# yemam3/SAC-RCBF

Hardware: AMD Instinct MI355X
Metric: safe env steps/sec (dynamics+CBF-QP) at batch 65536, 1/2/4/8 MI355X (higher is better)
Workload: dtype f32 rows / f64 QP / f64 env

## Files before the change

### __graft_entry__.py

```python
import os
import subprocess
import sys

ROOT = os.path.dirname(os.path.abspath(__file__))
PKG = os.path.join(ROOT, "sac-rcbf_amd")
CSRC = os.path.join(PKG, "csrc")
LIB = os.path.join(PKG, "rcbf_amd", "librcbf_hip.so")
HIPCC = os.environ.get("HIPCC", "/opt/rocm/bin/hipcc")
HIP_FLAGS = ["--offload-arch=gfx950", "-O3", "-fPIC", "-std=c++17",
             "-fhip-fp32-correctly-rounded-divide-sqrt", "-Wno-unused-result",
             "-mllvm", "-amdgpu-kernarg-preload-count=16"]

for p in (ROOT, PKG):
    if p not in sys.path:
        sys.path.insert(0, p)


def _newer(target, sources):
    if not os.path.exists(target):
        return False
    t = os.path.getmtime(target)
    return all(os.path.getmtime(s) <= t for s in sources)


KERNEL_TUS = ["rcbf_qp.hip", "rcbf_qp_f64.hip", "rcbf_qp_bwd.hip", "rcbf_layer.hip", "rcbf_env.hip", "rcbf_cascade.hip",
              "rcbf_gp.hip", "rcbf_model.hip", "rcbf_aql.hip", "rcbf_steps_traj.hip", "rcbf_steps_term.hip", "rcbf_policy.hip"]
TU_FLAGS = {"rcbf_steps_term.hip": ["-mllvm", "-disable-machine-licm"]}
LLVM_BIN = "/opt/rocm/lib/llvm/bin"
STEPS_CO = os.path.join(PKG, "rcbf_amd", "librcbf_steps.co")
STEPS_TRAJ_CO = os.path.join(PKG, "rcbf_amd", "librcbf_steps_traj.co")
STEPS_TERM_CO = os.path.join(PKG, "rcbf_amd", "librcbf_steps_term.co")
POLICY_CO = os.path.join(PKG, "rcbf_amd", "librcbf_policy.co")


def _deps(path, seen=None):
    import re
    seen = set() if seen is None else seen
    if path in seen or not os.path.exists(path):
        return seen
    seen.add(path)
    for name in re.findall(r'^\s*#\s*include\s+"([^"]+)"', open(path).read(), re.M):
        for d in (os.path.dirname(path), CSRC, os.path.join(ROOT, "include")):
            cand = os.path.normpath(os.path.join(d, name))
            if os.path.exists(cand):
                _deps(cand, seen)
                break
    return seen
# ... 14 lines not shown
        obj = os.path.join(objdir, tu.replace(".hip", ".o"))
        objs.append(obj)
        if not force and _newer(obj, sorted(_deps(src))):
            continue
        cmd = [HIPCC, *HIP_FLAGS, *TU_FLAGS.get(tu, []), *defines, *inc, "-c", "-o", obj, src]
        print("[build]", " ".join(cmd), flush=True)
        procs.append(subprocess.Popen(cmd))
    if any(p.wait() != 0 for p in procs):
        raise RuntimeError("hipcc failed")
    open(flags_file, "w").write(flags)
    if out == LIB:
        extract_steps_co(os.path.join(objdir, "rcbf_env.o"), STEPS_CO)
        extract_steps_co(os.path.join(objdir, "rcbf_steps_traj.o"), STEPS_TRAJ_CO)
        extract_steps_co(os.path.join(objdir, "rcbf_steps_term.o"), STEPS_TERM_CO)
        extract_steps_co(os.path.join(objdir, "rcbf_policy.o"), POLICY_CO)
    if not procs and _newer(out, objs):
        return out
    cmd = [HIPCC, "--offload-arch=gfx950", "-shared", "-fPIC", "-o", out, *objs, "-L/opt/rocm/lib", "-lhsa-runtime64"]
    print("[build]", " ".join(cmd), flush=True)
    subprocess.run(cmd, check=True)
    return out


def extract_steps_co(obj, out):
    if _newer(out, [obj]):
        return out
    import tempfile
    with tempfile.TemporaryDirectory() as td:
        fat = os.path.join(td, "fatbin.bin")
        subprocess.run([os.path.join(LLVM_BIN, "llvm-objcopy"), "--dump-section=.hip_fatbin=" + fat, obj,
# ... 158 lines not shown
    print("[smoke] ok", flush=True)


if __name__ == "__main__":
    what = sys.argv[1] if len(sys.argv) > 1 else "build"
    if what == "variant":
        name, defs = sys.argv[2], sys.argv[3:]
        os.makedirs(os.path.join(ROOT, "build", "variants"), exist_ok=True)
        vdir = os.path.join(ROOT, "build", "variants")
        build_lib(force=True, out=os.path.join(vdir, f"librcbf_{name}.so"), defines=defs)
        objdir = os.path.join(ROOT, "build", "obj_" + "_".join(d.strip("-D").replace("=", "") for d in defs))
        extract_steps_co(os.path.join(objdir, "rcbf_env.o"), os.path.join(vdir, f"librcbf_{name}.co"))
        extract_steps_co(os.path.join(objdir, "rcbf_steps_traj.o"), os.path.join(vdir, f"librcbf_{name}_traj.co"))
        extract_steps_co(os.path.join(objdir, "rcbf_steps_term.o"), os.path.join(vdir, f"librcbf_{name}_term.co"))
        extract_steps_co(os.path.join(objdir, "rcbf_policy.o"), os.path.join(vdir, f"librcbf_{name}_policy.co"))
    else:
        {"build": build, "smoke": smoke, "build_oracle": lambda: build_oracle(force=True)}[what]()
```

### include/rcbf_hip.h

```cpp
#ifndef RCBF_HIP_H
#define RCBF_HIP_H

#include <stdint.h>
#include <hip/hip_runtime_api.h>

#ifdef __cplusplus
extern "C" {
#endif

#define RCBF_ABI_VERSION 13

#define RCBF_MODE_SIMULATED_CARS 0
#define RCBF_MODE_UNICYCLE 1

#define RCBF_FORM_DIFF 0
#define RCBF_FORM_CASCADE 1

#define RCBF_SOLVER_ACTIVE_SET 0
#define RCBF_SOLVER_PDIPM 1
#define RCBF_SOLVER_GI 2

#define RCBF_QP_OK 0
#define RCBF_QP_MAX_ITER 1
#define RCBF_QP_INFEASIBLE 2
// ... 228 lines not shown
#define RCBF_TRAJ_U 2
#define RCBF_TRAJ_REWARD 4
#define RCBF_TRAJ_COST 8
#define RCBF_TRAJ_DONE 16
#define RCBF_TRAJ_GOAL_MET 32
#define RCBF_TRAJ_STATUS 64
#define RCBF_TRAJ_TERM_OBS 128
#define RCBF_AQL_PROFILE 1
#define RCBF_AQL_FIRST_ACQUIRE_SYSTEM 2
#define RCBF_AQL_LAST_RELEASE_AGENT 4
#define RCBF_AQL_STUDY_MID_NOFENCE 8
#define RCBF_AQL_STUDY_MID_NOACQ 16
#define RCBF_AQL_STUDY_MID_NOREL 32
#define RCBF_AQL_PROFILE_ENDS 64
#define RCBF_AQL_PER_STEP 128
#define RCBF_AQL_SAFE_STEP_KERNARG_BYTES 408
#define RCBF_AQL_SAFE_STEPS_KERNARG_BYTES 408
#define RCBF_AQL_SAFE_STEPS_TRAJ_KERNARG_BYTES 424
#define RCBF_AQL_SAFE_STEPS_TERM_KERNARG_BYTES 432
#define RCBF_AQL_POLICY_STEP_KERNARG_BYTES 80
typedef struct rcbf_aql rcbf_aql;
typedef struct rcbf_aql_plan rcbf_aql_plan;
int rcbf_aql_open(int32_t device, const char* code_object, int32_t flags, rcbf_aql** out);
int rcbf_aql_close(rcbf_aql* q);
int rcbf_aql_kernel_count(const rcbf_aql* q);
int rcbf_aql_safe_step_plan(rcbf_aql* q, const rcbf_params* prm, int64_t B, int32_t K, double* x, double* aux,
                            int32_t* step, uint32_t* episode, const float* const* u_rl_seq, int32_t n_u_rl,
                            const float* mu, const float* sigma, int32_t prior_cols, float* obs_out, float* u_out,
                            float* reward, float* cost, uint8_t* done, uint8_t* goal_met, int32_t* status_out,
                            int32_t* fail_flag, int32_t auto_reset, uint64_t seed, int64_t env_offset,
// ... 12 lines not shown
                                 int32_t* status_out, int32_t* fail_flag, int32_t auto_reset, uint64_t seed,
                                 int64_t env_offset, uint64_t* span_out, int32_t flags, int32_t traj_mask,
                                 int64_t traj_pitch, float* term_obs, rcbf_aql_plan** out);
int rcbf_aql_closed_loop_plan(rcbf_aql* q, const rcbf_params* prm, int64_t B, int32_t K, double* x, double* aux,
                              int32_t* step, uint32_t* episode, float* u_rl_buf, const float* mu, const float* sigma,
                              int32_t prior_cols, float* obs_out, float* u_out, float* reward, float* cost,
                              uint8_t* done, uint8_t* goal_met, int32_t* status_out, int32_t* fail_flag,
                              int32_t auto_reset, uint64_t seed, int64_t env_offset, uint64_t* span_out,
                              int32_t flags, int32_t traj_mask, int64_t traj_pitch, float* term_obs,
                              const float* obs_in, const float* packed, int32_t n_o, int32_t n_u, int32_t hidden,
                              int32_t mode, uint64_t policy_seed, const uint64_t* counter_word,
                              int64_t policy_env_offset, rcbf_aql_plan** out);
int rcbf_aql_run(rcbf_aql_plan* plan, uint64_t timeout_us);
int rcbf_aql_plan_times(const rcbf_aql_plan* plan, uint64_t* start_end_ns);
int rcbf_aql_plan_dispatches(const rcbf_aql_plan* plan);
int rcbf_aql_plan_free(rcbf_aql_plan* plan);

#define RCBF_POLICY_MEAN 0
#define RCBF_POLICY_SAMPLE 1
int64_t rcbf_policy_packed_floats(int32_t n_o, int32_t n_u, int32_t hidden);
int rcbf_policy_act(const float* packed, int32_t n_o, int32_t n_u, int32_t hidden, int64_t B,
                    const float* obs, float* u_rl, int32_t mode, const float* z,
                    uint64_t seed, uint64_t counter, int64_t env_offset, hipStream_t stream);

const char* rcbf_version(void);
int32_t rcbf_abi_version(void);
int32_t rcbf_params_size(void);

#ifdef __cplusplus
}
// ... 3 lines not shown
```

### sac-rcbf_amd/csrc/rcbf_aql.hip

```cpp
#include <hip/hip_runtime.h>
#include <hsa/hsa.h>
#include <hsa/hsa_ext_amd.h>

#include <dlfcn.h>
#include <immintrin.h>
#include <time.h>

#include <atomic>
#include <cstddef>
#include <cstdio>
#include <cstring>
#include <string>
#include <vector>

#include "rcbf_hip.h"
#include "rcbf_policy_step.hpp"
#include "rcbf_safe_step.hpp"

namespace {

using namespace rcbf;

struct SafeStepArgs {
    int64_t B;
// ... 53 lines not shown
struct rcbf_aql {
    int device = -1;
    hsa_agent_t agent{};
    hsa_queue_t* queue = nullptr;
    hsa_code_object_reader_t reader{};
    hsa_code_object_reader_t reader_traj{};
    hsa_executable_t exe{};
    hsa_executable_t exe_traj{};
    hsa_code_object_reader_t reader_term{};
    hsa_executable_t exe_term{};
    bool have_reader = false, have_reader_traj = false, have_exe = false, have_exe_traj = false, hsa_up = false;
    bool have_reader_term = false, have_exe_term = false;
    hsa_code_object_reader_t reader_policy{};
    hsa_executable_t exe_policy{};
    bool have_reader_policy = false, have_exe_policy = false;
    std::vector<char> code, code_traj, code_term, code_policy;
    std::vector<KernelInfo> kernels;
    std::atomic<int> queue_error{0};
    int profiling = 0;
    bool fused = false;
    bool traj = false;
    bool term = false;
    bool policy = false;
};

struct rcbf_aql_plan {
    rcbf_aql* q = nullptr;
    int device = -1;
    int32_t K = 0;
    void* kernargs = nullptr;
    std::vector<hsa_kernel_dispatch_packet_t> pkt;
    std::vector<hsa_signal_t> sig;
    int profiled = 0;
};

namespace {

void queue_error_cb(hsa_status_t status, hsa_queue_t*, void* data) {
    auto* q = static_cast<rcbf_aql*>(data);
    q->queue_error.store((int)status);
}

struct AgentSearch {
    uint32_t bdf;
    uint32_t domain;
    hsa_agent_t found{};
    bool ok = false;
};
// ... 46 lines not shown
std::string safe_steps_prefix(int mode, int k, int bs) {
    char buf[128];
    snprintf(buf, sizeof buf, "_ZN4rcbf12k_safe_stepsILi%dELi%dELi%dEEEv", mode, k, bs);
    return buf;
}

std::string safe_steps_traj_prefix(int mode, int k, int bs) {
    char buf[128];
    snprintf(buf, sizeof buf, "_ZN4rcbf17k_safe_steps_trajILi%dELi%dELi%dEEEv", mode, k, bs);
    return buf;
}

std::string safe_steps_term_prefix(int mode, int k, int bs) {
    char buf[128];
    snprintf(buf, sizeof buf, "_ZN4rcbf17k_safe_steps_termILi%dELi%dELi%dEEEv", mode, k, bs);
    return buf;
}

std::string policy_step_prefix(bool sample, int nrb) {
    char buf[128];
    snprintf(buf, sizeof buf, "_ZN4rcbf13k_policy_stepILb%dELi%dEEEv", sample ? 1 : 0, nrb);
    return buf;
}

bool read_optional_code_object(const std::string& tpath, std::vector<char>& code);

bool read_side_code_object(const std::string& path, const char* suffix, std::vector<char>& code) {
    if (path.size() <= 3 || path.compare(path.size() - 3, 3, ".co") != 0) return true;
    return read_optional_code_object(path.substr(0, path.size() - 3) + suffix + ".co", code);
}
// ... 98 lines not shown
        if (hipGetDevice(&prev) != hipSuccess) prev = -1;
        if (prev != dev) (void)hipSetDevice(dev);
    }
    ~DeviceGuard() {
        if (prev >= 0) (void)hipSetDevice(prev);
    }
};

void destroy(rcbf_aql* q) {
    if (!q) return;
    if (q->queue) hsa_queue_destroy(q->queue);
    if (q->have_exe) hsa_executable_destroy(q->exe);
    if (q->have_exe_traj) hsa_executable_destroy(q->exe_traj);
    if (q->have_exe_term) hsa_executable_destroy(q->exe_term);
    if (q->have_exe_policy) hsa_executable_destroy(q->exe_policy);
    if (q->have_reader_policy) hsa_code_object_reader_destroy(q->reader_policy);
    if (q->have_reader) hsa_code_object_reader_destroy(q->reader);
    if (q->have_reader_traj) hsa_code_object_reader_destroy(q->reader_traj);
    if (q->have_reader_term) hsa_code_object_reader_destroy(q->reader_term);
    if (q->hsa_up) hsa_shut_down();
    delete q;
}

}

extern "C" {

int rcbf_aql_open(int32_t device, const char* code_object_path, int32_t flags, rcbf_aql** out) {
    if (!out) return RCBF_E_NULL;
    *out = nullptr;
// ... 21 lines not shown
    const bool read_ok = n > 0 && fread(q->code.data(), 1, (size_t)n, f) == (size_t)n;
    fclose(f);
    if (!read_ok) {
        delete q;
        return RCBF_E_BAD_SHAPE;
    }
    if (!read_side_code_object(path, "_traj", q->code_traj)) {
        delete q;
        return RCBF_E_BAD_SHAPE;
    }
    if (!read_side_code_object(path, "_term", q->code_term)) {
        delete q;
        return RCBF_E_BAD_SHAPE;
    }
    if (!read_optional_code_object(policy_code_object_path(path), q->code_policy)) {
        delete q;
        return RCBF_E_BAD_SHAPE;
    }
    int rc = hsa_rc(hsa_init());
    if (rc) {
        delete q;
        return rc;
    }
    q->hsa_up = true;
    hipDeviceProp_t prop;
    if (hipGetDeviceProperties(&prop, device) != hipSuccess) {
        destroy(q);
        return RCBF_E_HSA;
    }
    AgentSearch s{(uint32_t)((prop.pciBusID << 8) | (prop.pciDeviceID << 3)), (uint32_t)prop.pciDomainID};
// ... 42 lines not shown
    }
    if (!rc && !q->code_policy.empty()) {
        rc = hsa_rc(hsa_code_object_reader_create_from_memory(q->code_policy.data(), q->code_policy.size(),
                                                              &q->reader_policy));
        if (!rc) q->have_reader_policy = true;
        if (!rc)
            rc = hsa_rc(hsa_executable_create_alt(HSA_PROFILE_FULL, HSA_DEFAULT_FLOAT_ROUNDING_MODE_DEFAULT, nullptr,
                                                  &q->exe_policy));
        if (!rc) q->have_exe_policy = true;
        if (!rc)
            rc = hsa_rc(
                hsa_executable_load_agent_code_object(q->exe_policy, q->agent, q->reader_policy, nullptr, nullptr));
        if (!rc) rc = hsa_rc(hsa_executable_freeze(q->exe_policy, nullptr));
        if (!rc) rc = hsa_rc(hsa_executable_iterate_agent_symbols(q->exe_policy, q->agent, collect_kernel, q));
    }
    int n_steps = 0, n_fused = 0, n_traj = 0, n_term = 0;
    for (const auto& k : q->kernels) {
        if (k.name.compare(0, 21, "_ZN4rcbf11k_safe_step") == 0) {
            ++n_steps;
            if (k.kernarg_bytes != sizeof(SafeStepArgs) || k.private_bytes != 0) rc = RCBF_E_BAD_SHAPE;
        } else if (k.name.compare(0, 22, "_ZN4rcbf12k_safe_steps") == 0) {
            ++n_fused;
            if (k.kernarg_bytes != sizeof(SafeStepsArgs) || k.private_bytes != 0) rc = RCBF_E_BAD_SHAPE;
        } else if (k.name.compare(0, 27, "_ZN4rcbf17k_safe_steps_traj") == 0) {
            ++n_traj;
            if (k.kernarg_bytes != sizeof(SafeStepsTrajArgs) || k.private_bytes != 0) rc = RCBF_E_BAD_SHAPE;
        } else if (k.name.compare(0, 27, "_ZN4rcbf17k_safe_steps_term") == 0) {
            ++n_term;
            if (k.kernarg_bytes != sizeof(SafeStepsTermArgs) || k.private_bytes != 0) rc = RCBF_E_BAD_SHAPE;
        }
    }
    if (!rc && n_steps == 0) rc = RCBF_E_BAD_MODE;
    q->fused = n_fused > 0;
    q->traj = n_traj > 0;
    q->term = n_term > 0;
    int n_policy = 0;
    for (int s = 0; s < 2; ++s)
        for (int nrb = 1; nrb <= 2; ++nrb) {
            const KernelInfo* kp = find_kernel(q, policy_step_prefix(s != 0, nrb));
            if (kp && kp->kernarg_bytes == sizeof(PolicyStepArgs) && kp->private_bytes == 0) ++n_policy;
        }
    q->policy = n_policy == 4;
    if (!rc)
        rc = hsa_rc(hsa_queue_create(q->agent, kQueueSize, HSA_QUEUE_TYPE_SINGLE, queue_error_cb, q, UINT32_MAX,
                                     UINT32_MAX, &q->queue));
    if (!rc && q->profiling) rc = hsa_rc(hsa_amd_profiling_set_profiler_enabled(q->queue, 1));
    if (rc) {
        destroy(q);
        return rc;
    }
// ... 92 lines not shown
                       {u_out, ext(row_u, nu * n * 4)},
                       {reward, ext(row_rew, n * 4)},
                       {cost, ext(row_cost, n * 4)},
                       {done, ext(row_done, n)},
                       {goal_met, ext(row_goal, n)},
                       {status_out, ext(row_stat, n * 4)},
                       {term_obs, ext(row_term, 0)},
                       {fail_flag, 4}};
        for (int32_t j = 0; j < n_u_rl && kf; ++j)
            for (const auto& w : written)
                if (overlaps(u_rl_seq[j], nu * n * 4, w.p, w.bytes)) {
                    kf = nullptr;
                    break;
                }
    }
    if (term && !kf) return RCBF_E_BAD_MODE;
    const int32_t npkt = kf ? (K + kFusedChunk - 1) / kFusedChunk : K;

    auto* p = new rcbf_aql_plan();
    p->q = q;
    p->device = q->device;
    p->K = K;
    p->profiled = ends ? 2 : profiled ? 1 : 0;
    const size_t table_off = (size_t)npkt * kArgStride;
    std::vector<unsigned char> host(table_off + (kf ? (size_t)n_u_rl * sizeof(const float*) : 0), 0);
    int rc = (int)hipMalloc(&p->kernargs, host.size());
    if (kf) std::memcpy(host.data() + table_off, u_rl_seq, (size_t)n_u_rl * sizeof(const float*));
    for (int32_t j = 0; j < npkt && !rc; ++j) {
        const int64_t r0 = kf ? (int64_t)j * kFusedChunk : (int64_t)j;
        if (kf) {
            SafeStepsTermArgs ea;
            std::memset(&ea, 0, sizeof ea);
            SafeStepsTrajArgs& ta = ea.t;
            SafeStepsArgs& a = ta.s;
            ea.term_obs = rows_on(term_obs, r0, row_term);
            ta.traj_mask = traj_mask;
            ta.traj_pitch = traj_pitch;
            io.fill(a, r0);
// ... 373 lines not shown
        if (hsa_amd_profiling_get_dispatch_time(p->q->agent, sg, &t) != HSA_STATUS_SUCCESS) return RCBF_E_HSA;
        if (p->profiled == 2 && p->K == 1 && p->sig.size() > 1) {
            hsa_amd_profiling_dispatch_time_t t2;
            if (hsa_amd_profiling_get_dispatch_time(p->q->agent, p->sig.back(), &t2) != HSA_STATUS_SUCCESS)
                return RCBF_E_HSA;
            t.end = t2.end;
        }
        start_end_ns[2 * j] = (uint64_t)((long double)t.start * 1e9L / (long double)freq);
        start_end_ns[2 * j + 1] = (uint64_t)((long double)t.end * 1e9L / (long double)freq);
    }
    return 0;
}

int rcbf_aql_plan_dispatches(const rcbf_aql_plan* p) { return p ? (int)p->pkt.size() : RCBF_E_NULL; }

int rcbf_aql_plan_free(rcbf_aql_plan* p) {
    if (!p) return 0;
    if (p->kernargs) {
        DeviceGuard guard(p->device);
        (void)hipFree(p->kernargs);
    }
    for (auto& s : p->sig) hsa_signal_destroy(s);
    delete p;
    return 0;
}

}
```

### sac-rcbf_amd/csrc/rcbf_device.hpp

```cpp
#pragma once

#include <hip/hip_runtime.h>
#include <stdint.h>

#include "rcbf_hip.h"

namespace rcbf {

constexpr double kInf = __builtin_huge_val();


#ifdef RCBF_STUDY_QP_STAMPS
__device__ __forceinline__ void qp_stamp(int j) {
    __builtin_amdgcn_sched_barrier(0);
    unsigned long long t;
    asm volatile("s_memtime %0\n\ts_waitcnt lgkmcnt(0)" : "=s"(t)::"memory");
    __builtin_amdgcn_sched_barrier(0);
    if ((threadIdx.x & 63) == 0 && rcbf_qp_stamp_buf)
        rcbf_qp_stamp_buf[((int64_t)blockIdx.x * 4 + (threadIdx.x >> 6)) * 16 + j] = t;
}
__device__ __forceinline__ void qp_count(int j, bool f) {
    const unsigned long long n = __popcll(__ballot(f));
    if ((threadIdx.x & 63) == 0 && rcbf_qp_stamp_buf)
        rcbf_qp_stamp_buf[((int64_t)blockIdx.x * 4 + (threadIdx.x >> 6)) * 16 + j] = n;
// ... 159 lines not shown
            for (int k = c; k < N; ++k) A[r][k] -= f * A[c][k];
            b[r] -= f * b[c];
        }
    }
#pragma unroll
    for (int i = N - 1; i >= 0; --i) {
        double v = b[i];
#pragma unroll
        for (int k = i + 1; k < N; ++k) v -= A[i][k] * x[k];
        x[i] = v * pinv[i];
    }
}

__device__ __forceinline__ float div_f32_via_rcp(float a, double rb) { return (float)((double)a * rb); }

__device__ __forceinline__ double sin_small(double x) {
    if (!(fabs(x) <= 1.3)) return sin(x);
    const double x2 = x * x;
    double p = -1.9572941063391263e-20;
    p = fma(p, x2, 8.2206352466243297e-18);
    p = fma(p, x2, -2.8114572543455206e-15);
    p = fma(p, x2, 7.6471637318198164e-13);
    p = fma(p, x2, -1.6059043836821613e-10);
    p = fma(p, x2, 2.5052108385441720e-08);
    p = fma(p, x2, -2.7557319223985893e-06);
    p = fma(p, x2, 1.9841269841269841e-04);
    p = fma(p, x2, -8.3333333333333332e-03);
    p = fma(p, x2, 1.6666666666666666e-01);
    return fma(-x * x2, p, x);
}

template <int N, bool DIAG>
// ... 1511 lines not shown
            G[r0][k] = (k == c2) ? 1.0 : 0.0;
            G[r0 + 1][k] = (k == c2) ? -1.0 : 0.0;
        }
        h[r0] = prm.u_max[c2] - u[c2];
        h[r0 + 1] = -prm.u_min[c2] + u[c2];
    }
}

struct CarsStepOut {
    float reward;
    double reward_d;
    double cost;
    bool done;
};

__device__ __forceinline__ double cars_env_pre(const rcbf_params& prm, double* xs, double& t, int& step,
                                               CarsStepOut& o) {
#pragma clang fp contract(off)
    const double kp = prm.kp, kb = prm.k_brake, dt = 0.02;
    double vdes0 = 30.0 - 10.0 * sin_small(0.2 * t);
    double acc[5];
    acc[0] = kp * (vdes0 - xs[1]);
#pragma unroll
    for (int i = 1; i < 5; ++i) acc[i] = kp * (30.0 - xs[2 * i + 1]);
    double d01 = xs[0] - xs[2], d12 = xs[2] - xs[4], d24 = xs[4] - xs[8];
    acc[1] += (-kb * d01) * (d01 < 6.0 ? 1.0 : 0.0);
    acc[2] += (-kb * d12) * (d12 < 6.0 ? 1.0 : 0.0);
    acc[4] += (-kb * d24) * (d24 < 13.0 ? 1.0 : 0.0);
#pragma unroll
    for (int i = 0; i < 5; ++i) acc[i] *= 1.1;
    double v[5];
#pragma unroll
    for (int i = 0; i < 5; ++i) v[i] = xs[2 * i + 1];
#pragma unroll
    for (int i = 0; i < 5; ++i) {
        xs[2 * i] += dt * v[i];
        if (i != 3) xs[2 * i + 1] += dt * acc[i];
    }
    t = t + dt;
    step += 1;
    o.done = step >= 300;
    double cost = 0.0;
    if (xs[4] - xs[6] < 2.99) cost -= 0.1;
    if (xs[6] - xs[8] < 2.99) cost -= 0.1;
    o.cost = cost;
    return acc[3];
}

template <typename A>
__device__ __forceinline__ void cars_env_post(double* xs, double acc3, A action, CarsStepOut& o) {
#pragma clang fp contract(off)
    const double dt = 0.02;
    const double gu = 50.0 * (double)action;
    xs[7] += dt * (acc3 + gu);
    A a2 = action * action;
    A r = (A)(-5.0) * (a2 < (A)0 ? -a2 : a2) / (A)300;
    o.reward = (float)r;
    o.reward_d = (double)r;
}

template <typename A>
__device__ __forceinline__ void cars_env_step(const rcbf_params& prm, double* xs, double& t, int& step, A action,
                                              CarsStepOut& o) {
    const double acc3 = cars_env_pre(prm, xs, t, step, o);
    cars_env_post<A>(xs, acc3, action, o);
}

__device__ __forceinline__ double div_const(double x, double d, double inv_d) {
    double q = x * inv_d;
    double r = fma(-q, d, x);
// ... 168 lines not shown
```

### sac-rcbf_amd/rcbf_amd/_lib.py

```python
import ctypes
import os
import warnings

import torch

_HERE = os.path.dirname(os.path.abspath(__file__))
LIB_PATH = os.environ.get("RCBF_HIP_LIB", os.path.join(_HERE, "librcbf_hip.so"))

MODE_SIMULATED_CARS = 0
MODE_UNICYCLE = 1
FORM_DIFF = 0
FORM_CASCADE = 1
SOLVER_ACTIVE_SET = 0
SOLVER_PDIPM = 1
SOLVER_GI = 2
POLICY_MEAN = 0
POLICY_SAMPLE = 1
QP_OK, QP_MAX_ITER, QP_INFEASIBLE, QP_NONFINITE = 0, 1, 2, 3
MAX_HAZARDS = 8
ABI_VERSION = 13

_ERRORS = {1001: "RCBF_E_BAD_MODE", 1002: "RCBF_E_BAD_SHAPE", 1003: "RCBF_E_NULL", 1004: "RCBF_E_HSA",
           1005: "RCBF_E_TIMEOUT", 1006: "RCBF_E_GP_HANDOFF"}

# ... 97 lines not shown
                                  _P, _I32, _U64, _I64, _P, _I32, _I32, _I64, _P, _P, _P, _I32, _I32, _I32, _I32,
                                  _U64, _P, _I64, ctypes.POINTER(ctypes.c_void_p)],
    "rcbf_traj_pack_replay_f64": [_P, _I64, _I64, _I64, _I32, _I64, _I32, _I32, _P, _P, _P, _P, _P, _P, _P, _I32,
                                  ctypes.c_double, _I32, _P],
    "rcbf_traj_pack_gp_f64": [_P, _P, _P, _P, _I64, _I32, _I64, _I32, _I32, _P, _P, _P, _P, _P, _P, ctypes.c_double,
                              _I32, _I32, _I64, _P],
    "rcbf_traj_pack_gp_scratch_bytes": [_I64, _I32],
    "rcbf_traj_episode_stats_f64": [_P, _P, _P, _P, _P, _P, _P, _I64, _I32, _I64, _P, _P, _P, _P, _P, _P, _P, _I32,
                                    _I64, _P],
    "rcbf_traj_episode_stats_scratch_bytes": [_I64, _I32],
    "rcbf_policy_act": [_P, _I32, _I32, _I32, _I64, _P, _P, _I32, _P, _U64, _U64, _I64, _P],
    "rcbf_policy_packed_floats": [_I32, _I32, _I32],
    "rcbf_aql_run": [_P, _U64],
    "rcbf_aql_plan_times": [_P, _P],
    "rcbf_aql_plan_dispatches": [_P],
    "rcbf_aql_plan_free": [_P],
    "rcbf_host_free": [_P],
    "rcbf_version": [],
    "rcbf_abi_version": [],
    "rcbf_params_size": [],
}

_lib = None
_load_error = None


def load():
    global _lib, _load_error
    if _lib is not None:
        return _lib
# ... 100 lines not shown
```

### sac-rcbf_amd/rcbf_amd/aql.py

```python
import ctypes
import weakref

import torch

from . import _lib

PROFILE = 1
PROFILE_ENDS = 64
PER_STEP = 128
TRAJ_OBS, TRAJ_U, TRAJ_REWARD, TRAJ_COST, TRAJ_DONE, TRAJ_GOAL_MET, TRAJ_STATUS = 1, 2, 4, 8, 16, 32, 64
TRAJ_BITS = {"obs": TRAJ_OBS, "u": TRAJ_U, "reward": TRAJ_REWARD, "cost": TRAJ_COST, "done": TRAJ_DONE,
             "goal_met": TRAJ_GOAL_MET, "status": TRAJ_STATUS}
TRAJ_TERM_OBS = 128


def _bind():
    return _lib.load()


def _check(rc, what):
    _lib.check(rc, what)


class AqlQueue:
# ... 16 lines not shown
    def handle(self):
        if not self._fin.alive:
            raise RuntimeError("the AQL queue is closed")
        return self._h

    def kernel_count(self):
        return int(_lib.load().rcbf_aql_kernel_count(self.handle))

    def close(self):
        for p in list(self._plans):
            p.free()
        self._fin()

    def safe_step_plan(self, env, u_rl_seq, layer, steps=None, mean=None, sigma=None, outputs=None,
                       auto_reset=True, prior_layout="rows", span=None, profile=False, fence_flags=0, fused=None,
                       trajectory=None):
        if env.device != self.device:
            raise ValueError(f"env on {env.device}, queue on {self.device}")
        o = outputs if outputs is not None else env.make_outputs()
        us = [env._u_arg(u) for u in u_rl_seq]
        if not us:
            raise ValueError("u_rl_seq is empty")
        K = len(us) if steps is None else int(steps)
        if prior_layout not in ("rows", "cols"):
            raise ValueError(f"prior_layout must be 'rows' or 'cols', got {prior_layout!r}")
        cols = prior_layout == "cols"
        if cols:
            if mean is not None and env.dynamics_mode == "SimulatedCars":
                raise ValueError("the cars CBF rows read no mean (diff_cbf_qp.py:298-299): pass mean=None")
            mean, sigma = env._prior_cols_arg(mean, "mean"), env._prior_cols_arg(sigma, "sigma")
        else:
            mean, sigma = env._prior_arg(mean, "mean"), env._prior_arg(sigma, "sigma")
        if span is not None:
            nw = (env.num_envs + 63) // 64
            if not (torch.is_tensor(span) and span.dtype == torch.int64 and span.device == env.device
                    and span.is_contiguous() and span.numel() >= 4 * nw * K):
                raise ValueError(f"span must be a contiguous int64 tensor of >= {4 * nw * K} entries "
                                 f"(K blocks of ceil(B / 64) x 4) on {env.device}")
        a = env._step_args(layer, o, auto_reset)
        arr = (ctypes.c_void_p * len(us))(*[u.data_ptr() for u in us])
        h = ctypes.c_void_p()
        flags = (PROFILE if profile else 0) | (PER_STEP if fused is False else 0) | int(fence_flags)
        head = (self.handle, ctypes.byref(layer._prm), env.num_envs, K, *[v or None for v in a[2:6]], arr, len(us),
                None if mean is None else mean.data_ptr(), None if sigma is None else sigma.data_ptr(), int(cols))
        tail = (*a[17:20], None if span is None else span.data_ptr(), flags)
        traj = None
        if trajectory is not None and trajectory is not False:
            if span is not None:
                raise ValueError("a trajectory plan takes no span buffer")
            traj = env.make_trajectory(K) if trajectory is True else dict(trajectory)
            mask, pitch = _trajectory_args(env, traj, K)
            term = traj.get("term_obs")
            if term is not None:
                why = _term_plan_refusal(env, layer, us, term, K, pitch, profile, fused, fence_flags)
                if why:
                    raise ValueError(f"a trajectory plan with term_obs is always fused, but {why}")
            outs = list(a[9:17])
# ... 151 lines not shown
            o = self._keep[2]
            for f, t in self.trajectory.items():
                if f == "term_obs":
                    continue
                dst = self._env.obs if f == "obs" else o.get(f)
                if dst is not None and not (f == "goal_met" and self._env.dynamics_mode == "SimulatedCars"):
                    dst.copy_(t[self.K - 1])
        return self._env.obs, self._keep[2]["reward"], self._keep[2]["done"], self._keep[2]

    @property
    def dispatches(self):
        if not self._fin.alive:
            raise RuntimeError("the AQL plan was freed")
        return int(_lib.load().rcbf_aql_plan_dispatches(self._h))

    def times_ns(self):
        import numpy as np
        if not self._fin.alive or not self.queue._fin.alive:
            raise RuntimeError("the AQL plan (or its queue) was freed")
        out = np.zeros((self.K, 2), dtype=np.uint64)
        _check(_lib.load().rcbf_aql_plan_times(self._h, out.ctypes.data), "rcbf_aql_plan_times")
        return out.astype(np.int64)

    def free(self):
        self._fin()


class ClosedLoopPlan(AqlPlan):

    def __init__(self, queue, handle, K, keep, env, trajectory, policy, u_rl, word):
# ... 25 lines not shown
```

Before: 53.30 billion.

## Add fast fused cars multi-step kernel with polynomial sine and paired steps

Adds a specialised fused multi-step kernel for the SimulatedCars mode. It is selected by default when no trajectory, goal_met or status outputs are requested. Whenever the whole wave's time argument stays inside the polynomial range, it skips the sin range-check branch, processes two steps per loop iteration with software-prefetched actions, uses reciprocal multiply for the reward, and writes obs with full-wave float4 stores. Otherwise it falls back to the generic step body. The cost is another code object and loader path, plus more special-case code that must stay numerically equivalent to the original.

```diff
diff --git a/__graft_entry__.py b/__graft_entry__.py
--- a/__graft_entry__.py
+++ b/__graft_entry__.py
@@ -24,13 +24,15 @@
 
 
 KERNEL_TUS = ["rcbf_qp.hip", "rcbf_qp_f64.hip", "rcbf_qp_bwd.hip", "rcbf_layer.hip", "rcbf_env.hip", "rcbf_cascade.hip",
-              "rcbf_gp.hip", "rcbf_model.hip", "rcbf_aql.hip", "rcbf_steps_traj.hip", "rcbf_steps_term.hip", "rcbf_policy.hip"]
+              "rcbf_gp.hip", "rcbf_model.hip", "rcbf_aql.hip", "rcbf_steps_traj.hip", "rcbf_steps_term.hip", "rcbf_policy.hip",
+              "rcbf_steps_fast.hip"]
 TU_FLAGS = {"rcbf_steps_term.hip": ["-mllvm", "-disable-machine-licm"]}
 LLVM_BIN = "/opt/rocm/lib/llvm/bin"
 STEPS_CO = os.path.join(PKG, "rcbf_amd", "librcbf_steps.co")
 STEPS_TRAJ_CO = os.path.join(PKG, "rcbf_amd", "librcbf_steps_traj.co")
 STEPS_TERM_CO = os.path.join(PKG, "rcbf_amd", "librcbf_steps_term.co")
 POLICY_CO = os.path.join(PKG, "rcbf_amd", "librcbf_policy.co")
+STEPS_FAST_CO = os.path.join(PKG, "rcbf_amd", "librcbf_steps_fast.co")
 
 
 def _deps(path, seen=None):
@@ -75,6 +77,7 @@
         extract_steps_co(os.path.join(objdir, "rcbf_steps_traj.o"), STEPS_TRAJ_CO)
         extract_steps_co(os.path.join(objdir, "rcbf_steps_term.o"), STEPS_TERM_CO)
         extract_steps_co(os.path.join(objdir, "rcbf_policy.o"), POLICY_CO)
+        extract_steps_co(os.path.join(objdir, "rcbf_steps_fast.o"), STEPS_FAST_CO)
     if not procs and _newer(out, objs):
         return out
     cmd = [HIPCC, "--offload-arch=gfx950", "-shared", "-fPIC", "-o", out, *objs, "-L/opt/rocm/lib", "-lhsa-runtime64"]
@@ -263,5 +266,6 @@
         extract_steps_co(os.path.join(objdir, "rcbf_steps_traj.o"), os.path.join(vdir, f"librcbf_{name}_traj.co"))
         extract_steps_co(os.path.join(objdir, "rcbf_steps_term.o"), os.path.join(vdir, f"librcbf_{name}_term.co"))
         extract_steps_co(os.path.join(objdir, "rcbf_policy.o"), os.path.join(vdir, f"librcbf_{name}_policy.co"))
+        extract_steps_co(os.path.join(objdir, "rcbf_steps_fast.o"), os.path.join(vdir, f"librcbf_{name}_fast.co"))
     else:
         {"build": build, "smoke": smoke, "build_oracle": lambda: build_oracle(force=True)}[what]()
diff --git a/include/rcbf_hip.h b/include/rcbf_hip.h
--- a/include/rcbf_hip.h
+++ b/include/rcbf_hip.h
@@ -266,6 +266,10 @@
 #define RCBF_AQL_STUDY_MID_NOREL 32
 #define RCBF_AQL_PROFILE_ENDS 64
 #define RCBF_AQL_PER_STEP 128
+#define RCBF_AQL_FUSED_LOOP 256
+#define RCBF_AQL_FORM_PER_STEP 0
+#define RCBF_AQL_FORM_FUSED 1
+#define RCBF_AQL_FORM_FUSED_FAST 2
 #define RCBF_AQL_SAFE_STEP_KERNARG_BYTES 408
 #define RCBF_AQL_SAFE_STEPS_KERNARG_BYTES 408
 #define RCBF_AQL_SAFE_STEPS_TRAJ_KERNARG_BYTES 424
@@ -308,6 +312,7 @@
 int rcbf_aql_run(rcbf_aql_plan* plan, uint64_t timeout_us);
 int rcbf_aql_plan_times(const rcbf_aql_plan* plan, uint64_t* start_end_ns);
 int rcbf_aql_plan_dispatches(const rcbf_aql_plan* plan);
+int rcbf_aql_plan_form(const rcbf_aql_plan* plan);
 int rcbf_aql_plan_free(rcbf_aql_plan* plan);
 
 #define RCBF_POLICY_MEAN 0
diff --git a/sac-rcbf_amd/csrc/rcbf_aql.hip b/sac-rcbf_amd/csrc/rcbf_aql.hip
--- a/sac-rcbf_amd/csrc/rcbf_aql.hip
+++ b/sac-rcbf_amd/csrc/rcbf_aql.hip
@@ -91,13 +91,17 @@
     hsa_code_object_reader_t reader_policy{};
     hsa_executable_t exe_policy{};
     bool have_reader_policy = false, have_exe_policy = false;
-    std::vector<char> code, code_traj, code_term, code_policy;
+    hsa_code_object_reader_t reader_fast{};
+    hsa_executable_t exe_fast{};
+    bool have_reader_fast = false, have_exe_fast = false;
+    std::vector<char> code, code_traj, code_term, code_policy, code_fast;
     std::vector<KernelInfo> kernels;
     std::atomic<int> queue_error{0};
     int profiling = 0;
     bool fused = false;
     bool traj = false;
     bool term = false;
+    bool fast = false;
     bool policy = false;
 };
 
@@ -109,6 +113,7 @@
     std::vector<hsa_kernel_dispatch_packet_t> pkt;
     std::vector<hsa_signal_t> sig;
     int profiled = 0;
+    int form = RCBF_AQL_FORM_PER_STEP;
 };
 
 namespace {
@@ -185,6 +190,12 @@
 std::string safe_steps_term_prefix(int mode, int k, int bs) {
     char buf[128];
     snprintf(buf, sizeof buf, "_ZN4rcbf17k_safe_steps_termILi%dELi%dELi%dEEEv", mode, k, bs);
+    return buf;
+}
+
+std::string safe_steps_fast_prefix(int bs) {
+    char buf[128];
+    snprintf(buf, sizeof buf, "_ZN4rcbf17k_safe_steps_fastILi%dEEEv", bs);
     return buf;
 }
 
@@ -313,6 +324,8 @@
     if (q->have_exe_traj) hsa_executable_destroy(q->exe_traj);
     if (q->have_exe_term) hsa_executable_destroy(q->exe_term);
     if (q->have_exe_policy) hsa_executable_destroy(q->exe_policy);
+    if (q->have_exe_fast) hsa_executable_destroy(q->exe_fast);
+    if (q->have_reader_fast) hsa_code_object_reader_destroy(q->reader_fast);
     if (q->have_reader_policy) hsa_code_object_reader_destroy(q->reader_policy);
     if (q->have_reader) hsa_code_object_reader_destroy(q->reader);
     if (q->have_reader_traj) hsa_code_object_reader_destroy(q->reader_traj);
@@ -364,6 +377,10 @@
         return RCBF_E_BAD_SHAPE;
     }
     if (!read_optional_code_object(policy_code_object_path(path), q->code_policy)) {
+        delete q;
+        return RCBF_E_BAD_SHAPE;
+    }
+    if (!read_side_code_object(path, "_fast", q->code_fast)) {
         delete q;
         return RCBF_E_BAD_SHAPE;
     }
@@ -436,6 +453,20 @@
         if (!rc) rc = hsa_rc(hsa_executable_freeze(q->exe_policy, nullptr));
         if (!rc) rc = hsa_rc(hsa_executable_iterate_agent_symbols(q->exe_policy, q->agent, collect_kernel, q));
     }
+    if (!rc && !q->code_fast.empty()) {
+        rc = hsa_rc(
+            hsa_code_object_reader_create_from_memory(q->code_fast.data(), q->code_fast.size(), &q->reader_fast));
+        if (!rc) q->have_reader_fast = true;
+        if (!rc)
+            rc = hsa_rc(hsa_executable_create_alt(HSA_PROFILE_FULL, HSA_DEFAULT_FLOAT_ROUNDING_MODE_DEFAULT, nullptr,
+                                                  &q->exe_fast));
+        if (!rc) q->have_exe_fast = true;
+        if (!rc)
+            rc = hsa_rc(
+                hsa_executable_load_agent_code_object(q->exe_fast, q->agent, q->reader_fast, nullptr, nullptr));
+        if (!rc) rc = hsa_rc(hsa_executable_freeze(q->exe_fast, nullptr));
+        if (!rc) rc = hsa_rc(hsa_executable_iterate_agent_symbols(q->exe_fast, q->agent, collect_kernel, q));
+    }
     int n_steps = 0, n_fused = 0, n_traj = 0, n_term = 0;
     for (const auto& k : q->kernels) {
         if (k.name.compare(0, 21, "_ZN4rcbf11k_safe_step") == 0) {
@@ -456,6 +487,12 @@
     q->fused = n_fused > 0;
     q->traj = n_traj > 0;
     q->term = n_term > 0;
+    int n_fast = 0;
+    for (int bs : {64, 128, 256}) {
+        const KernelInfo* kp = find_kernel(q, safe_steps_fast_prefix(bs));
+        if (kp && kp->kernarg_bytes == sizeof(SafeStepsArgs) && kp->private_bytes == 0) ++n_fast;
+    }
+    q->fast = n_fast == 3;
     int n_policy = 0;
     for (int s = 0; s < 2; ++s)
         for (int nrb = 1; nrb <= 2; ++nrb) {
@@ -578,6 +615,15 @@
                     break;
                 }
     }
+    bool fast = false;
+    if (kf && q->fast && cars && !term && !traj_mask && K > 1 && B % 64 == 0 && !(((uintptr_t)obs_out) & 15) &&
+        !goal_met && !status_out && episode && fail_flag && !(flags & RCBF_AQL_FUSED_LOOP)) {
+        const KernelInfo* kfast = find_kernel(q, safe_steps_fast_prefix(bs));
+        if (kfast && kfast->kernarg_bytes == sizeof(SafeStepsArgs)) {
+            kf = kfast;
+            fast = true;
+        }
+    }
     if (term && !kf) return RCBF_E_BAD_MODE;
     const int32_t npkt = kf ? (K + kFusedChunk - 1) / kFusedChunk : K;
 
@@ -586,6 +632,7 @@
     p->device = q->device;
     p->K = K;
     p->profiled = ends ? 2 : profiled ? 1 : 0;
+    p->form = fast ? RCBF_AQL_FORM_FUSED_FAST : kf ? RCBF_AQL_FORM_FUSED : RCBF_AQL_FORM_PER_STEP;
     const size_t table_off = (size_t)npkt * kArgStride;
     std::vector<unsigned char> host(table_off + (kf ? (size_t)n_u_rl * sizeof(const float*) : 0), 0);
     int rc = (int)hipMalloc(&p->kernargs, host.size());
@@ -989,6 +1036,8 @@
 
 int rcbf_aql_plan_dispatches(const rcbf_aql_plan* p) { return p ? (int)p->pkt.size() : RCBF_E_NULL; }
 
+int rcbf_aql_plan_form(const rcbf_aql_plan* p) { return p ? p->form : RCBF_E_NULL; }
+
 int rcbf_aql_plan_free(rcbf_aql_plan* p) {
     if (!p) return 0;
     if (p->kernargs) {
diff --git a/sac-rcbf_amd/csrc/rcbf_device.hpp b/sac-rcbf_amd/csrc/rcbf_device.hpp
--- a/sac-rcbf_amd/csrc/rcbf_device.hpp
+++ b/sac-rcbf_amd/csrc/rcbf_device.hpp
@@ -197,8 +197,11 @@
 
 __device__ __forceinline__ float div_f32_via_rcp(float a, double rb) { return (float)((double)a * rb); }
 
+template <bool POLY_ONLY = false>
 __device__ __forceinline__ double sin_small(double x) {
-    if (!(fabs(x) <= 1.3)) return sin(x);
+    if constexpr (!POLY_ONLY) {
+        if (!(fabs(x) <= 1.3)) return sin(x);
+    }
     const double x2 = x * x;
     double p = -1.9572941063391263e-20;
     p = fma(p, x2, 8.2206352466243297e-18);
@@ -1740,11 +1743,12 @@
     bool done;
 };
 
+template <bool POLY_ONLY = false>
 __device__ __forceinline__ double cars_env_pre(const rcbf_params& prm, double* xs, double& t, int& step,
                                                CarsStepOut& o) {
 #pragma clang fp contract(off)
     const double kp = prm.kp, kb = prm.k_brake, dt = 0.02;
-    double vdes0 = 30.0 - 10.0 * sin_small(0.2 * t);
+    double vdes0 = 30.0 - 10.0 * sin_small<POLY_ONLY>(0.2 * t);
     double acc[5];
     acc[0] = kp * (vdes0 - xs[1]);
 #pragma unroll
@@ -1773,13 +1777,20 @@
     return acc[3];
 }
 
-template <typename A>
+template <typename A, bool RCP = false>
 __device__ __forceinline__ void cars_env_post(double* xs, double acc3, A action, CarsStepOut& o) {
 #pragma clang fp contract(off)
     const double dt = 0.02;
     const double gu = 50.0 * (double)action;
     xs[7] += dt * (acc3 + gu);
     A a2 = action * action;
+    if constexpr (RCP) {
+        static_assert(sizeof(A) == 4, "div_f32_via_rcp: fp32 operands");
+        const float r = div_f32_via_rcp((float)((A)(-5.0) * (a2 < (A)0 ? -a2 : a2)), 1.0 / 300.0);
+        o.reward = r;
+        o.reward_d = (double)r;
+        return;
+    }
     A r = (A)(-5.0) * (a2 < (A)0 ? -a2 : a2) / (A)300;
     o.reward = (float)r;
     o.reward_d = (double)r;
diff --git a/sac-rcbf_amd/csrc/rcbf_safe_steps_fast.hpp b/sac-rcbf_amd/csrc/rcbf_safe_steps_fast.hpp
--- /dev/null
+++ b/sac-rcbf_amd/csrc/rcbf_safe_steps_fast.hpp
@@ -0,0 +1,292 @@
+#pragma once
+
+#include "rcbf_safe_step.hpp"
+
+#ifndef RCBF_FAST_PAIR
+#define RCBF_FAST_PAIR 1
+#endif
+#ifndef RCBF_FAST_AHEAD2
+#define RCBF_FAST_AHEAD2 1
+#endif
+
+namespace rcbf {
+
+__device__ __forceinline__ void seed_off_from_kernargs(uint32_t koff, uint64_t& seed, int64_t& off) {
+    seed = 0;
+    off = 0;
+#if defined(__HIP_DEVICE_COMPILE__)
+    typedef const char __attribute__((address_space(4)))* cbytes_t;
+    const cbytes_t ka = (cbytes_t)__builtin_amdgcn_kernarg_segment_ptr() + koff;
+    seed = *reinterpret_cast<const uint64_t __attribute__((address_space(4)))*>(ka + offsetof(SafeStepsArgs, seed));
+    off = *reinterpret_cast<const int64_t __attribute__((address_space(4)))*>(ka + offsetof(SafeStepsArgs, off));
+#endif
+}
+
+__device__ __forceinline__ void store_obs_chunks_full(gptr<float> obs, int64_t base, const float* lds_wave, int lane) {
+    constexpr int NO = Dims<RCBF_MODE_SIMULATED_CARS, 1>::NO;
+    static_assert(NO * 16 == 2 * 64 + 32, "two whole rounds and half a round of chunks");
+    __builtin_amdgcn_wave_barrier();
+    const float4* src = reinterpret_cast<const float4*>(lds_wave);
+    const gptr<float> dst = obs + base * NO;
+    const int c2 = 128 + (lane & 31);
+    const float4 k0 = src[lane], k1 = src[64 + lane], k2 = src[c2];
+    st_out4<false>(dst + 4 * lane, k0);
+    st_out4<false>(dst + 4 * (64 + lane), k1);
+    st_out4<false>(dst + 4 * c2, k2);
+}
+
+struct CarsFastHead {
+    LayerState<RCBF_MODE_SIMULATED_CARS, 1> L;
+    double acc3;
+    float u_rl, cst;
+    bool dn;
+};
+
+__device__ __forceinline__ void cars_fast_head(const rcbf_params& prm, double* xs, double& a, int& st, float u_rl,
+                                               const float* m, const float* s, const float* obs_c, CarsFastHead& h) {
+    constexpr int MODE = RCBF_MODE_SIMULATED_CARS;
+    using D = Dims<MODE, 1>;
+    const float us[1] = {u_rl};
+    float s32[D::NS];
+    state_from_obs32<MODE>(obs_c, s32);
+    diff_rows<MODE, 1>(prm, s32, us, m, s, h.L.G, h.L.h, nullptr);
+    CarsStepOut o;
+    h.acc3 = cars_env_pre<true>(prm, xs, a, st, o);
+    h.dn = o.done;
+    h.cst = (float)o.cost;
+    h.u_rl = u_rl;
+}
+
+__device__ __forceinline__ void cars_fast_mid(const rcbf_params& prm, int64_t B, int64_t i, gptr<double> x,
+                                              gptr<double> aux, gptr<int32_t> step, gptr<uint32_t> episode,
+                                              gptr<float> u_out, gptr<float> reward, gptr<float> cost,
+                                              gptr<uint8_t> done, int auto_reset, double* xs, double& a, int& st,
+                                              uint32_t& epr, float* obs_c, float* obs_stage, int lane, int& fail_bits,
+                                              CarsFastHead& h) {
+    constexpr int MODE = RCBF_MODE_SIMULATED_CARS;
+    using D = Dims<MODE, 1>;
+    const bool rs = auto_reset && h.dn;
+    if (__builtin_expect(rs, 0)) {
+        uint32_t koff = 0;
+        asm volatile("" : "+s"(koff));
+        uint64_t seed;
+        int64_t off;
+        seed_off_from_kernargs(koff, seed, off);
+        const uint32_t ep = epr + 1u;
+        episode[i] = ep;
+        epr = ep;
+        env_reset_one<MODE>(nullptr, i, seed, off, ep, xs, a, st);
+    }
+#pragma unroll
+    for (int p = 0; p < D::NS / 2; ++p)
+        if (p != 3) st_out2d(&x[2 * (p * B + i)], xs[2 * p], xs[2 * p + 1]);
+    st_out(&aux[i], a);
+    st_out(&step[i], st);
+    __builtin_amdgcn_sched_barrier(0);
+    const float us[1] = {h.u_rl};
+    float uf[1];
+    layer_solve_raw<MODE, 1>(prm, us, uf, h.L);
+    const int status = h.L.qp.status;
+    const double v3_reset = xs[7];
+    CarsStepOut o;
+    cars_env_post<float, true>(xs, h.acc3, uf[0], o);
+    xs[7] = rs ? v3_reset : xs[7];
+    st_out2d(&x[2 * (3 * B + i)], xs[6], xs[7]);
+    double ob[D::NO];
+    env_obs<MODE>(xs, ob);
+#pragma unroll
+    for (int k = 0; k < D::NO; ++k) obs_c[k] = (float)ob[k];
+#pragma unroll
+    for (int k = 0; k < D::NO / 2; ++k)
+        *reinterpret_cast<float2*>(&obs_stage[lane * D::NO + 2 * k]) = make_float2(obs_c[2 * k], obs_c[2 * k + 1]);
+    st_out(&u_out[i], uf[0]);
+    st_out(&reward[i], o.reward);
+    st_out(&cost[i], h.cst);
+    st_out(&done[i], (uint8_t)h.dn);
+    fail_bits |= status != RCBF_QP_OK ? 1 << status : 0;
+}
+
+__device__ __forceinline__ void cars_fast_chunks(int64_t i, gptr<double> x, gptr<double> aux, gptr<int32_t> step,
+                                                 gptr<float> obs_out, gptr<float> u_out, gptr<float> reward,
+                                                 gptr<float> cost, gptr<uint8_t> done, float* obs_stage, int lane) {
+    if constexpr (RCBF_FAST_PAIR != 0)
+        store_obs_chunks_full(obs_out, i - lane, obs_stage, lane);
+    else
+        store_obs_chunks<RCBF_MODE_SIMULATED_CARS, false, false, gptr<float>, false, true>(obs_out, i - lane,
+                                                                                           obs_stage, lane);
+    __builtin_amdgcn_wave_barrier();
+    asm volatile("" ::"s"(obs_out), "s"(x), "s"(aux), "s"(step), "s"(u_out), "s"(reward), "s"(cost), "s"(done) : "memory");
+}
+
+template <int BS = kBlock>
+__global__ void __launch_bounds__(BS) k_safe_steps_fast(
+    int64_t B, double* __restrict__ x, double* __restrict__ aux, int32_t* __restrict__ step,
+    const float* const* __restrict__ u_tab, uint32_t* __restrict__ episode, const float* __restrict__ mu,
+    const float* __restrict__ sigma, float* __restrict__ obs_out, float* __restrict__ u_out,
+    float* __restrict__ reward, float* __restrict__ cost, uint8_t* __restrict__ done, uint8_t* __restrict__ goal_met,
+    int32_t* __restrict__ status_out, int32_t* fail_flag, int auto_reset, uint64_t seed, int64_t off, rcbf_params prm,
+    int prior_cols, int n_u, int steps, int ju0) {
+    constexpr int MODE = RCBF_MODE_SIMULATED_CARS;
+    using D = Dims<MODE, 1>;
+    static_assert(D::NU == 1 && RCBF_EARLY_STORE && RCBF_FUSED_RAW_ROWS != 0, "the cars fused step's product form");
+    (void)goal_met;
+    (void)status_out;
+    const int64_t i = env_index<BS>();
+    if (i >= B) return;
+    double xs[D::NS];
+    load_state<MODE>(x, B, i, xs);
+    double a = ld_in(&aux[i]);
+    int st = ld_in(&step[i]);
+    typedef const uint64_t __attribute__((address_space(4)))* ctab_t;
+    const ctab_t tab = (ctab_t)reinterpret_cast<const uint64_t*>(u_tab);
+    auto next_j = [n_u](int j) { return j + 1 == n_u ? 0 : j + 1; };
+    static_assert(RCBF_FAST_AHEAD2 || !RCBF_FAST_PAIR, "the pair form loads two steps ahead");
+    float u0 = ld_in(&reinterpret_cast<gptr<const float>>(tab[ju0])[i]);
+    int ju = next_j(ju0);
+    float u1 = 0.0f;
+#if RCBF_FAST_AHEAD2
+    u1 = ld_in(&reinterpret_cast<gptr<const float>>(tab[ju])[i]);
+    ju = next_j(ju);
+#endif
+    uint64_t p2 = tab[ju], p3 = 0;
+#if RCBF_FAST_PAIR
+    ju = next_j(ju);
+    p3 = tab[ju];
+#endif
+    uint32_t epr = ld_in(&episode[i]);
+    prefetch_kernargs<7>();
+    float m[D::NS], s[D::NS];
+    if (prior_cols) {
+#pragma unroll
+        for (int k = 0; k < D::NS; ++k) {
+            m[k] = 0.0f;
+            s[k] = prior_sigma<MODE>(k);
+        }
+        if (sigma) {
+            s[5] = ld_in(&sigma[i]);
+            s[7] = ld_in(&sigma[B + i]);
+            s[9] = ld_in(&sigma[2 * B + i]);
+        }
+    } else {
+#pragma unroll
+        for (int k = 0; k < D::NS; ++k) {
+            m[k] = mu ? mu[i * D::NS + k] : 0.0f;
+            s[k] = sigma ? sigma[i * D::NS + k] : prior_sigma<MODE>(k);
+        }
+    }
+    __shared__ float obs_stage[BS / 64][64 * D::NO];
+    const gptr<double> xv = (gptr<double>)x;
+    const gptr<double> auxv = (gptr<double>)aux;
+    const gptr<int32_t> stepv = (gptr<int32_t>)step;
+    gptr<uint32_t> epv = (gptr<uint32_t>)episode;
+    const gptr<float> obsv = (gptr<float>)obs_out;
+    const gptr<float> uv = (gptr<float>)u_out;
+    const gptr<float> rewv = (gptr<float>)reward;
+    const gptr<float> costv = (gptr<float>)cost;
+    const gptr<uint8_t> donev = (gptr<uint8_t>)done;
+    gptr<int32_t> failv = (gptr<int32_t>)fail_flag;
+    const int lane = threadIdx.x & 63, wid = threadIdx.x >> 6;
+    int left = steps;
+    __builtin_amdgcn_s_waitcnt(0x0f70);
+    float obs_c[D::NO];
+    {
+        double o[D::NO];
+        env_obs<MODE>(xs, o);
+#pragma unroll
+        for (int k = 0; k < D::NO; ++k) obs_c[k] = (float)o[k];
+    }
+#define RCBF_FAST_WALK_HEAD()                                             \
+    const float un_ = ld_in(&reinterpret_cast<gptr<const float>>(p2)[i]); \
+    ju = next_j(ju);                                                      \
+    const uint64_t pn_ = tab[ju]
+#if RCBF_FAST_PAIR
+#define RCBF_FAST_WALK_TAIL() \
+    u0 = u1;                  \
+    u1 = un_;                 \
+    p2 = p3;                  \
+    p3 = pn_
+#elif RCBF_FAST_AHEAD2
+#define RCBF_FAST_WALK_TAIL() \
+    u0 = u1;                  \
+    u1 = un_;                 \
+    p2 = pn_
+#else
+#define RCBF_FAST_WALK_TAIL() \
+    u0 = un_;                 \
+    p2 = pn_
+#endif
+#define RCBF_FAST_MID(H_)                                                                                           \
+    cars_fast_mid(prm, B, i, xv, auxv, stepv, epv, uv, rewv, costv, donev, auto_reset, xs, a, st, epr, obs_c, \
+                  obs_stage[wid], lane, fail_bits, H_)
+#define RCBF_FAST_CHUNKS() cars_fast_chunks(i, xv, auxv, stepv, obsv, uv, rewv, costv, donev, obs_stage[wid], lane)
+    constexpr int PER = RCBF_FAST_PAIR ? 2 : 1;
+#pragma nounroll
+    while (left >= PER) {
+        bool in_range = fabs(0.2 * a) <= 1.3;
+        if (PER == 2) in_range = in_range && fabs(0.2 * (a + 0.02)) <= 1.3;
+        if (__builtin_amdgcn_ballot_w64(!in_range) != 0) break;
+        asm volatile("" : "+v"(epv), "+v"(failv));
+        int fail_bits = 0;
+        left -= PER;
+#if RCBF_FAST_PAIR
+        const float n0 = ld_in(&reinterpret_cast<gptr<const float>>(p2)[i]);
+        const float n1 = ld_in(&reinterpret_cast<gptr<const float>>(p3)[i]);
+        ju = next_j(ju);
+        const uint64_t q2 = tab[ju];
+        ju = next_j(ju);
+        const uint64_t q3 = tab[ju];
+        CarsFastHead ha, hb;
+        cars_fast_head(prm, xs, a, st, u0, m, s, obs_c, ha);
+        RCBF_FAST_MID(ha);
+        __builtin_amdgcn_sched_barrier(0);
+        cars_fast_head(prm, xs, a, st, u1, m, s, obs_c, hb);
+        __builtin_amdgcn_sched_barrier(0);
+        RCBF_FAST_CHUNKS();
+        RCBF_FAST_MID(hb);
+        RCBF_FAST_CHUNKS();
+        u0 = n0;
+        u1 = n1;
+        p2 = q2;
+        p3 = q3;
+#else
+        RCBF_FAST_WALK_HEAD();
+        CarsFastHead ha;
+        cars_fast_head(prm, xs, a, st, u0, m, s, obs_c, ha);
+        RCBF_FAST_MID(ha);
+        RCBF_FAST_CHUNKS();
+        RCBF_FAST_WALK_TAIL();
+#endif
+        if (__builtin_expect(fail_bits != 0, 0))
+            __hip_atomic_fetch_or(failv, fail_bits, __ATOMIC_RELAXED, __HIP_MEMORY_SCOPE_AGENT);
+    }
+    const Stamps<false> stamps{};
+#pragma nounroll
+    while (left > 0) {
+        --left;
+        asm volatile("" : "+v"(epv), "+v"(failv));
+        RCBF_FAST_WALK_HEAD();
+        const float us[1] = {u0};
+        bool rs = false;
+        safe_step_body<RCBF_SOLVER_ACTIVE_SET, MODE, 1, false, false, true, false, false, 1>(
+            prm, B, i, xv, auxv, stepv, epv, obsv, uv, rewv, costv, donev, (gptr<uint8_t>)nullptr,
+            (gptr<int32_t>)nullptr, failv, auto_reset, seed, off, xs, a, st, us, m, s, true, epr, stamps, obs_stage[wid],
+            nullptr, lane, &rs, obs_c);
+        epr += rs ? 1u : 0u;
+        __builtin_amdgcn_wave_barrier();
+        asm volatile("" ::: "memory");
+        RCBF_FAST_WALK_TAIL();
+    }
+#undef RCBF_FAST_MID
+#undef RCBF_FAST_CHUNKS
+#undef RCBF_FAST_WALK_HEAD
+#undef RCBF_FAST_WALK_TAIL
+}
+
+#define RCBF_SAFE_STEPS_FAST_INSTANTIATE(BS_)                                                                       \
+    template __global__ void k_safe_steps_fast<BS_>(                                                                \
+        int64_t, double* __restrict__, double* __restrict__, int32_t* __restrict__, const float* const* __restrict__, \
+        uint32_t* __restrict__, const float* __restrict__, const float* __restrict__, float* __restrict__,          \
+        float* __restrict__, float* __restrict__, float* __restrict__, uint8_t* __restrict__, uint8_t* __restrict__, \
+        int32_t* __restrict__, int32_t*, int, uint64_t, int64_t, rcbf_params, int, int, int, int)
+
+}
diff --git a/sac-rcbf_amd/csrc/rcbf_steps_fast.hip b/sac-rcbf_amd/csrc/rcbf_steps_fast.hip
--- /dev/null
+++ b/sac-rcbf_amd/csrc/rcbf_steps_fast.hip
@@ -0,0 +1,7 @@
+#include "rcbf_safe_steps_fast.hpp"
+
+namespace rcbf {
+RCBF_SAFE_STEPS_FAST_INSTANTIATE(64);
+RCBF_SAFE_STEPS_FAST_INSTANTIATE(128);
+RCBF_SAFE_STEPS_FAST_INSTANTIATE(256);
+}
diff --git a/sac-rcbf_amd/rcbf_amd/_lib.py b/sac-rcbf_amd/rcbf_amd/_lib.py
--- a/sac-rcbf_amd/rcbf_amd/_lib.py
+++ b/sac-rcbf_amd/rcbf_amd/_lib.py
@@ -135,6 +135,7 @@
     "rcbf_aql_run": [_P, _U64],
     "rcbf_aql_plan_times": [_P, _P],
     "rcbf_aql_plan_dispatches": [_P],
+    "rcbf_aql_plan_form": [_P],
     "rcbf_aql_plan_free": [_P],
     "rcbf_host_free": [_P],
     "rcbf_version": [],
diff --git a/sac-rcbf_amd/rcbf_amd/aql.py b/sac-rcbf_amd/rcbf_amd/aql.py
--- a/sac-rcbf_amd/rcbf_amd/aql.py
+++ b/sac-rcbf_amd/rcbf_amd/aql.py
@@ -8,6 +8,8 @@
 PROFILE = 1
 PROFILE_ENDS = 64
 PER_STEP = 128
+FUSED_LOOP = 256
+FORMS = ("per_step", "fused", "fused_fast")
 TRAJ_OBS, TRAJ_U, TRAJ_REWARD, TRAJ_COST, TRAJ_DONE, TRAJ_GOAL_MET, TRAJ_STATUS = 1, 2, 4, 8, 16, 32, 64
 TRAJ_BITS = {"obs": TRAJ_OBS, "u": TRAJ_U, "reward": TRAJ_REWARD, "cost": TRAJ_COST, "done": TRAJ_DONE,
              "goal_met": TRAJ_GOAL_MET, "status": TRAJ_STATUS}
@@ -54,7 +56,7 @@
 
     def safe_step_plan(self, env, u_rl_seq, layer, steps=None, mean=None, sigma=None, outputs=None,
                        auto_reset=True, prior_layout="rows", span=None, profile=False, fence_flags=0, fused=None,
-                       trajectory=None):
+                       trajectory=None, fast=None):
         if env.device != self.device:
             raise ValueError(f"env on {env.device}, queue on {self.device}")
         o = outputs if outputs is not None else env.make_outputs()
@@ -80,7 +82,8 @@
         a = env._step_args(layer, o, auto_reset)
         arr = (ctypes.c_void_p * len(us))(*[u.data_ptr() for u in us])
         h = ctypes.c_void_p()
-        flags = (PROFILE if profile else 0) | (PER_STEP if fused is False else 0) | int(fence_flags)
+        flags = ((PROFILE if profile else 0) | (PER_STEP if fused is False else 0) |
+                 (FUSED_LOOP if fast is False else 0) | int(fence_flags))
         head = (self.handle, ctypes.byref(layer._prm), env.num_envs, K, *[v or None for v in a[2:6]], arr, len(us),
                 None if mean is None else mean.data_ptr(), None if sigma is None else sigma.data_ptr(), int(cols))
         tail = (*a[17:20], None if span is None else span.data_ptr(), flags)
@@ -262,6 +265,12 @@
             raise RuntimeError("the AQL plan was freed")
         return int(_lib.load().rcbf_aql_plan_dispatches(self._h))
 
+    @property
+    def form(self):
+        if not self._fin.alive:
+            raise RuntimeError("the AQL plan was freed")
+        return FORMS[int(_lib.load().rcbf_aql_plan_form(self._h))]
+
     def times_ns(self):
         import numpy as np
         if not self._fin.alive or not self.queue._fin.alive:
```

Result: faster. 57.90 billion (median of 6 runs) (+8.6%).
